# Brochu/RayTrace-WE-GPU

Measured on AMD Instinct MI355X. Metric: Msamples/sec (pixels x spp) at 1920x1080 spp=100 depth=50, higher is better.
Workload: dtype f32

## Files before the change

### raytrace-we-gpu_amd/csrc/rtx_diag.h

```cpp
#pragma once

#include "rtx_internal.h"

#ifndef RTX_DIAG_PROF
#define RTX_DIAG_PROF 0
#endif
#ifndef RTX_DIAG_PIXEL
#define RTX_DIAG_PIXEL 0
#endif
#ifndef RTX_DIAG_COOP
#define RTX_DIAG_COOP 0
#endif
#ifndef RTX_DIAG_RAYS
#define RTX_DIAG_RAYS 0
#endif

namespace rtx {
namespace {

#if RTX_DIAG_PROF
__device__ __forceinline__ uint32_t *diag_slots() {
    __shared__ uint32_t s[4][8];
    return s[(threadIdx.x / 64) & 3u];
}
__device__ __forceinline__ void diag_add(int k, uint32_t v) {
    const uint64_t m = __ballot(1);
    if ((int)(threadIdx.x & 63u) == __ffsll((long long)m) - 1) diag_slots()[k] += v;
}
#define RTX_DIAG_ADD(k, v) diag_add(k, v)
#else
#define RTX_DIAG_ADD(k, v)
#endif

#define RTX_CP(k)                                                   \
    if (RTX_DIAG_COOP && cp) {                                      \
        const unsigned long long tn = __builtin_readcyclecounter(); \
        cp[k] += tn - *tq;                                          \
        *tq = tn;                                                   \
    }

struct Diag {
#if RTX_DIAG_RAYS
    uint32_t rit = 0;
#endif
#if RTX_DIAG_PROF
    unsigned long long pr[7] = {0, 0, 0, 0, 0, 0, 0};
    unsigned long long tq = 0;
#endif
#if RTX_DIAG_COOP
    unsigned long long cpa[8] = {0, 0, 0, 0, 0, 0, 0, 0};
    unsigned long long ctq = 0;
    bool was_coop = false;
#endif
    __device__ __forceinline__ void begin() {
#if RTX_DIAG_PROF
        if ((threadIdx.x & 63u) == 0u)
            for (int k = 0; k < 8; ++k) diag_slots()[k] = 0u;
        tq = __builtin_readcyclecounter();
#endif
#if RTX_DIAG_COOP
        ctq = __builtin_readcyclecounter();
#endif
    }
    __device__ __forceinline__ void section(int k) {
#if RTX_DIAG_PROF
        const unsigned long long tn = __builtin_readcyclecounter();
        pr[k] += tn - tq;
        tq = tn;
#else
        (void)k;
#endif
    }
    __device__ __forceinline__ void iteration(uint64_t act) {
#if RTX_DIAG_PROF
        pr[4]++;
        pr[6] += __popcll(act);
#else
        (void)act;
#endif
    }
    __device__ __forceinline__ void tail_iteration() {
#if RTX_DIAG_PROF
        pr[5]++;
#endif
    }
    __device__ __forceinline__ unsigned long long *coop_begin(uint32_t tier, unsigned long long *&tqp) {
#if RTX_DIAG_COOP
        tqp = &ctq;
        if (tier != (uint32_t)RTX_DIAG_COOP) return nullptr;
        const unsigned long long tn = __builtin_readcyclecounter();
        if (was_coop) cpa[4] += tn - ctq;
        ctq = tn;
        return cpa;
#else
        (void)tier;
        tqp = nullptr;
        return nullptr;
#endif
    }
    __device__ __forceinline__ void coop_end(unsigned long long *cp, uint32_t tier) {
#if RTX_DIAG_COOP
        if (cp) {
            const unsigned long long tn = __builtin_readcyclecounter();
            cpa[3] += tn - ctq;
            ctq = tn;
        }
        was_coop = tier == (uint32_t)RTX_DIAG_COOP;
#else
        (void)cp;
        (void)tier;
#endif
    }
    __device__ __forceinline__ void rays(const KParams &P, f3 o, f3 d, bool live, uint32_t slot) {
#if RTX_DIAG_RAYS
        if (!P.wave_times) return;
        const uint32_t w = blockIdx.x * (blockDim.x / 64u) + threadIdx.x / 64u;
        if ((++rit + w * 13u) % (uint32_t)RTX_DIAG_RAYS != 0u) return;
        unsigned long long r = 0;
        if ((threadIdx.x & 63u) == 0u) r = atomicAdd(&P.wave_times[0], 1ull);
        r = __shfl(r, 0, 64);
        const unsigned long long base = 64ull + 256ull * r;
        if (base + 256ull > 2ull * P.wave_cap) return;
        auto pk = [](float a, float b) {
            return ((unsigned long long)__float_as_uint(b) << 32) | __float_as_uint(a);
        };
        unsigned long long *q = P.wave_times + base + 4u * (threadIdx.x & 63u);
        q[0] = pk(o.x, o.y);
        q[1] = pk(o.z, d.x);
        q[2] = pk(d.y, d.z);
        q[3] = ((unsigned long long)slot << 32) | (live ? 1u : 0u);
#else
        (void)P, (void)o, (void)d, (void)live, (void)slot;
#endif
    }
    __device__ __forceinline__ void finish(const KParams &P) {
#if RTX_DIAG_PROF
        if (P.wave_times && (threadIdx.x & 63u) == 0u) {
            for (int k = 0; k < 7; ++k) atomicAdd(&P.wave_times[k], pr[k]);
            for (int k = 0; k < 7; ++k) atomicAdd(&P.wave_times[8 + k], (unsigned long long)diag_slots()[k]);
        }
#endif
#if RTX_DIAG_COOP
        if (P.wave_times && (threadIdx.x & 63u) == 0u)
            for (int k = 0; k < 6; ++k) atomicAdd(&P.wave_times[k], cpa[k]);
#endif
        (void)P;
    }
};

__device__ __forceinline__ void diag_pixel_start(const KParams &P, uint32_t gid, unsigned long long mode) {
#if RTX_DIAG_PIXEL
    if (P.wave_times && gid < P.wave_cap) P.wave_times[2 * gid] = (__builtin_amdgcn_s_memrealtime() << 2) | mode;
#else
    (void)P;
    (void)gid;
    (void)mode;
#endif
}
__device__ __forceinline__ void diag_pixel_end(const KParams &P, uint32_t gid) {
#if RTX_DIAG_PIXEL
    if (P.wave_times && gid < P.wave_cap) P.wave_times[2 * gid + 1] = __builtin_amdgcn_s_memrealtime();
#else
    (void)P;
    (void)gid;
#endif
}
constexpr bool kDiagAny = RTX_DIAG_PROF || RTX_DIAG_PIXEL || RTX_DIAG_COOP || RTX_DIAG_RAYS;

}
}
```

### raytrace-we-gpu_amd/csrc/rtx_grid.h

```cpp
#pragma once

#include <math.h>
#include <stdint.h>

#include <algorithm>
#include <cmath>
#include <utility>
#include <vector>

#if defined(__HIPCC__)
#define RTX_GD __host__ __device__ __forceinline__
#else
#define RTX_GD static inline
#endif

namespace rtx {

constexpr float kGridOMax = 64.0f;
constexpr double kGridFatCells = 1.0 / 256.0;
constexpr double kGridSlabPad = 1e-3;
#ifndef RTX_GRID_STEPS
#define RTX_GRID_STEPS 48
#endif
#ifndef RTX_GRID_HLOG
#define RTX_GRID_HLOG 0
#endif
constexpr uint32_t kGridMaxSteps = RTX_GRID_STEPS;
constexpr uint32_t kGridMaxCells = 4096;

struct LayerGrid {
    float x0, z0;
    float h, inv_h;
    float ylo, yhi;
    uint32_t nx, nz;
    float far_m;
    uint32_t nblk;
};

template <typename Visit>
RTX_GD bool grid_walk(const LayerGrid &G, uint32_t max_steps, float ox, float oy, float oz, float dx, float dy,
                      float dz, float t_stop, Visit visit) {
    const float o2 = fmaf(ox, ox, fmaf(oy, oy, oz * oz));
    const float d2 = fmaf(dx, dx, fmaf(dy, dy, dz * dz));
    if (!(o2 <= kGridOMax * kGridOMax) || !(d2 <= 3.0e38f)) return false;
    const float inf = INFINITY;
    float t0 = 0.0f, t1 = t_stop >= 0.0f ? t_stop : inf;
    auto clip = [&](float o, float d, float lo, float hi) {
        if (d == 0.0f) {
            if (!(o >= lo && o <= hi)) t1 = -inf;
            return;
        }
        const float inv = 1.0f / d;
        const float ta = (lo - o) * inv, tb = (hi - o) * inv;
        t0 = fmaxf(t0, fminf(ta, tb));
        t1 = fminf(t1, fmaxf(ta, tb));
    };
    clip(oy, dy, G.ylo, G.yhi);
    clip(ox, dx, G.x0, G.x0 + (float)G.nx * G.h);
    clip(oz, dz, G.z0, G.z0 + (float)G.nz * G.h);
    if (!(t0 <= t1)) return true;
    const float sx = (fmaf(t0, dx, ox) - G.x0) * G.inv_h, sz = (fmaf(t0, dz, oz) - G.z0) * G.inv_h;
    int ix = (int)fminf(fmaxf(floorf(sx), 0.0f), (float)(G.nx - 1));
    int iz = (int)fminf(fmaxf(floorf(sz), 0.0f), (float)(G.nz - 1));
    const int stx = dx > 0.0f ? 1 : -1, stz = dz > 0.0f ? 1 : -1;
    const float ivx = dx == 0.0f ? 0.0f : 1.0f / dx, ivz = dz == 0.0f ? 0.0f : 1.0f / dz;
    for (uint32_t k = 0; k < max_steps; ++k) {
        if (!visit((uint32_t)ix * G.nz + (uint32_t)iz)) return false;
        const float bx = fmaf((float)(ix + (dx > 0.0f ? 1 : 0)), G.h, G.x0);
        const float bz = fmaf((float)(iz + (dz > 0.0f ? 1 : 0)), G.h, G.z0);
        const float tx = dx == 0.0f ? inf : (bx - ox) * ivx;
        const float tz = dz == 0.0f ? inf : (bz - oz) * ivz;
        if (!(fminf(tx, tz) <= t1)) return true;
        if (tx <= tz) {
            ix += stx;
            if (ix < 0 || ix >= (int)G.nx) return true;
        } else {
            iz += stz;
            if (iz < 0 || iz >= (int)G.nz) return true;
        }
    }
    return false;
}

template <typename Cell>
RTX_GD uint64_t grid_mask(const LayerGrid &G, Cell cell, float ox, float oy, float oz, float dx, float dy, float dz,
                          float t_stop = INFINITY) {
    uint64_t m = 0ull;
    const bool done = grid_walk(G, kGridMaxSteps, ox, oy, oz, dx, dy, dz, t_stop, [&](uint32_t k) {
        m |= cell(k);
        return true;
    });
    return done ? m : ~0ull;
}

template <typename Add>
inline bool build_layer_grid_cells(const float *sph, uint32_t m, uint32_t max_cells, LayerGrid &G, Add add) {
    if (m == 0) return false;
    const double u = 5.9604644775390625e-08;
    const double y0 = sph[1];
    const double B = 26.0 * u * (double)kGridOMax * (double)kGridOMax;
    auto rho_of = [&](uint32_t j) {
        const double cx = sph[4 * (size_t)j], cz = sph[4 * (size_t)j + 2], r = sph[4 * (size_t)j + 3];
        const double c2 = cx * cx + y0 * y0 + cz * cz;
        return std::sqrt(r * r * (1.0 + 8.0 * u) + 27.0 * u * c2 + B) * (1.0 + 4.0 * u) * (1.0 + 1e-12);
    };
    double rho_max = 0.0, cmax = 0.0, xlo = INFINITY, xhi = -INFINITY, zlo = INFINITY, zhi = -INFINITY;
    for (uint32_t j = 0; j < m; ++j) {
        const double cx = sph[4 * (size_t)j], cz = sph[4 * (size_t)j + 2];
        const double rho = rho_of(j);
        rho_max = std::fmax(rho_max, rho);
        cmax = std::fmax(cmax, std::sqrt(cx * cx + y0 * y0 + cz * cz));
        xlo = std::fmin(xlo, cx - rho), xhi = std::fmax(xhi, cx + rho);
        zlo = std::fmin(zlo, cz - rho), zhi = std::fmax(zhi, cz + rho);
    }
    const double area = std::fmax((xhi - xlo) * (zhi - zlo), 1e-30);
    double h = std::exp2(std::round(std::log2(std::sqrt(area / m))) + RTX_GRID_HLOG);
    while (h < rho_max) h *= 2.0;
    const double fat = kGridFatCells * h;
    const double x0 = (std::floor((xlo - fat) / h) - 1.0) * h, z0 = (std::floor((zlo - fat) / h) - 1.0) * h;
    const double nxd = std::ceil((xhi + fat - x0) / h) + 1.0, nzd = std::ceil((zhi + fat - z0) / h) + 1.0;
    if (nxd * nzd > max_cells || !(std::fabs(x0) < 1e6 && std::fabs(z0) < 1e6)) return false;
    G.nx = (uint32_t)nxd, G.nz = (uint32_t)nzd;
    G.h = (float)h, G.inv_h = (float)(1.0 / h);
    G.x0 = (float)x0, G.z0 = (float)z0;
    const double slab = rho_max + kGridSlabPad;
    G.ylo = nextafterf((float)(y0 - slab), -INFINITY);
    G.yhi = nextafterf((float)(y0 + slab), INFINITY);
    G.far_m = nextafterf((float)(4e-3 * ((double)kGridOMax + cmax) + 1e-3), INFINITY);
    for (uint32_t j = 0; j < m; ++j) {
        const double cx = sph[4 * (size_t)j], cz = sph[4 * (size_t)j + 2];
        const double rho = rho_of(j) + fat;
        const int ax = (int)std::floor((cx - rho - x0) / h), bxi = (int)std::floor((cx + rho - x0) / h);
        const int az = (int)std::floor((cz - rho - z0) / h), bzi = (int)std::floor((cz + rho - z0) / h);
        for (int ix = std::max(ax, 0); ix <= std::min(bxi, (int)G.nx - 1); ++ix)
            for (int iz = std::max(az, 0); iz <= std::min(bzi, (int)G.nz - 1); ++iz) {
                const double qx = std::fmin(std::fmax(cx, x0 + ix * h), x0 + (ix + 1) * h);
                const double qz = std::fmin(std::fmax(cz, z0 + iz * h), z0 + (iz + 1) * h);
                if ((qx - cx) * (qx - cx) + (qz - cz) * (qz - cz) <= rho * rho) add((uint32_t)ix * G.nz + iz, j);
            }
    }
    return true;
}

template <typename Vec>
inline bool build_layer_grid(const float *sph, uint32_t i_lo, uint32_t i_hi, LayerGrid &G, Vec &cell) {
    const uint32_t m = i_hi - i_lo;
    if (m == 0 || (m + 7) / 8 > 64) return false;
    std::vector<std::pair<uint32_t, uint32_t>> hits;
    if (!build_layer_grid_cells(sph + 4 * (size_t)i_lo, m, kGridMaxCells, G,
                                [&](uint32_t k, uint32_t j) { hits.emplace_back(k, j); }))
        return false;
    G.nblk = (m + 7) / 8;
    cell.assign((size_t)G.nx * G.nz, 0ull);
    for (const auto &h : hits) cell[h.first] |= 1ull << (h.second / 8);
    return true;
}

}
```

### raytrace-we-gpu_amd/csrc/rtx_kernels.hip

```cpp
#include <algorithm>
#include <cstdlib>
#include <cstring>
#include <mutex>
#include <type_traits>
#include <vector>

#include "rtx_device_math.h"
#include "rtx_diag.h"
#include "rtx_internal.h"
#include "rtx_prefilter.h"

#if defined(__HIP_DEVICE_COMPILE__) && !defined(__gfx950__)
#error "rtx_kernels.hip targets gfx950 (MI355X) only"
#endif

namespace rtx {

namespace {

constexpr float kTMin = 0.001f;

struct FrameVals {
    f3 org, hor, ver, llc;
    float img_w, img_h;
// ... 383 lines not shown
__device__ __forceinline__ uint32_t scan_prefilter(cfloat_p pre, uint32_t b, uint32_t nblk, const LineTest &T,
                                                   const KScene &S, uint32_t *list, uint32_t &cnt,
                                                   uint32_t *pack = nullptr, const float *lds_pr = nullptr,
                                                   uint64_t gm = ~0ull) {
    cnt = 0;
    uint32_t *my = list + threadIdx.x;
    const LineFlat K = line_test_flat(T, S.flat_cy);
    while (b < nblk) {
        bool full;
        if (b < S.flat_lo) {
            b = scan_range<kPF, false, kTile>(pre, b, min(S.flat_lo, nblk), T, T.nou, T.nov, my, cnt, full, pack, lds_pr);
        } else if (b < S.flat_hi) {
            b = scan_range<kPF, true, kTile>(pre, b, min(S.flat_hi, nblk), T, K.ku, K.kv, my, cnt, full, pack, lds_pr,
                                             gm, S.flat_lo);
        } else {
            b = scan_range<kPF, false, kTile>(pre, b, nblk, T, T.nou, T.nov, my, cnt, full, pack, lds_pr);
        }
        if (full) break;
    }
    return b;
}

__device__ __forceinline__ uint64_t hit_key(float best, int idx) {
    return ((uint64_t)__float_as_uint(best) << 32) | (uint32_t) ~(uint32_t)(idx + 1);
}
__device__ __forceinline__ void key_hit(uint64_t k, float &best, int &idx) {
    best = __uint_as_float((uint32_t)(k >> 32));
    idx = (int)~(uint32_t)k - 1;
}

__device__ __forceinline__ void resolve_one(float4 sc, int g, bool live, f3 o, f3 d, float a, float inv_a,
                                            float t_min, uint64_t &key, bool &ok) {
    const float inf = __uint_as_float(0x7f800000u);
    const float ocx = o.x - sc.x;
    const float ocy = o.y - sc.y;
    const float ocz = o.z - sc.z;
    const float hb = fmaf(ocz, d.z, fmaf(ocy, d.y, ocx * d.x));
    const float cc = fmaf(ocz, ocz, fmaf(ocy, ocy, fmaf(ocx, ocx, -(sc.w * sc.w))));
    const float disc = fmaf(hb, hb, -(a * cc));
    const bool cand = live & !(disc < 0.0f);
    const float sq = sqrt_rn(disc);
    const float rn = (-hb - sq) * inv_a;
    const float rf = (-hb + sq) * inv_a;
    const bool fin = fabsf(rn) < inf && fabsf(rf) < inf;
    ok = ok & (!cand | fin);
    const float c = !(rn < t_min) ? rn : rf;
    const uint64_t k = ((uint64_t)__float_as_uint(c) << 32) | (uint32_t) ~(uint32_t)(g + 1);
    const bool acc = cand & !(c < t_min) & (k < key);
    key = acc ? k : key;
}

struct GiIdentity {
    __device__ __forceinline__ uint32_t operator()(uint32_t p) const { return p; }
};
template <typename Ld, typename Gi = GiIdentity, bool kPos = false>
__device__ __forceinline__ bool resolve_pre_t(Ld ld, uint32_t n, const uint32_t *list, uint32_t m, f3 o, f3 d,
                                              float a, float inv_a, float t_min, float &best, int &idx,
                                              uint32_t cap = (uint32_t)kCand, Gi gi = Gi()) {
    bool ok = true;
    uint32_t j = 0;
    uint32_t e = list[threadIdx.x];
    RTX_DIAG_ADD(4, (uint32_t)__popcll(__ballot(m != 0u)));
#if RTX_DIAG_PROF
    {
        uint32_t c = 0;
        for (uint32_t q = 0; q < m; ++q) c += (uint32_t)__popc(list[min(q, cap) * kRB + threadIdx.x] >> 24);
#pragma unroll
        for (int off = 32; off > 0; off >>= 1) c += (uint32_t)__shfl_xor((int)c, off, 64);
        RTX_DIAG_ADD(5, c);
    }
#endif
    uint32_t pos = 0;
    auto next = [&](uint32_t &i, bool &live) {
        live = j < m;
        pos = (e & 0xffffffu) + (uint32_t)__builtin_ctz(live ? (e >> 24) : 1u);
        if constexpr (kPos) pos = min(pos, n - 1u);
        i = gi(pos);
        e &= e - (1u << 24);
        const bool adv = live && (e >> 24) == 0u;
        j += adv ? 1u : 0u;
        const uint32_t nx = list[min(j, cap) * kRB + threadIdx.x];
        e = adv ? nx : e;
    };
    uint32_t i0;
    bool l0;
    next(i0, l0);
    float4 v0 = kPos ? ld(pos) : ld(min(i0, n - 1u));
    uint64_t key = hit_key(best, idx);
    while (__ballot(l0) != 0ull) {
        RTX_DIAG_ADD(2, 1u);
        uint32_t i1;
        bool l1;
        next(i1, l1);
        const float4 v1 = kPos ? ld(pos) : ld(min(i1, n - 1u));
        resolve_one(v0, (int)i0, l0, o, d, a, inv_a, t_min, key, ok);
        i0 = i1;
        l0 = l1;
        v0 = v1;
    }
    key_hit(key, best, idx);
    return ok;
}
__device__ __forceinline__ bool resolve_pre(const float4 *__restrict__ cen, uint32_t n, const uint32_t *list,
                                            uint32_t m, f3 o, f3 d, float a, float inv_a, float t_min,
                                            float &best, int &idx) {
    return resolve_pre_t([cen](uint32_t i) { return cen[i]; }, n, list, m, o, d, a, inv_a, t_min, best, idx);
}

__device__ __forceinline__ uint32_t scan_culled(const KScene &S, uint32_t b, const LineTest &T, const LineTest &Ts,
                                                const HalfTest &H, const HalfTest &Hs, uint32_t *list,
                                                uint32_t &cnt) {
    cnt = 0;
    uint32_t *my = list + threadIdx.x;
    const uint32_t nblk = S.n_cpad / 8u;
    const LineFlat K = line_test_flat(T, S.flat_cy);
    const LineFlat Ks = line_test_flat(Ts, kCullSy * S.flat_cy);
    const f2v uxs = {Ts.ux, Ts.ux}, uzs = {Ts.uz, Ts.uz}, vzs = {Ts.vz, Ts.vz}, kus = {Ks.ku, Ks.ku},
              kvs = {Ks.kv, Ks.kv};
    const float thr_bs = Ts.thr * kCullThrScaleSy;
    f2v ux = {T.ux, T.ux}, uy = {T.uy, T.uy}, uz = {T.uz, T.uz}, vy = {T.vy, T.vy}, vz = {T.vz, T.vz};
    f2v ku = {K.ku, K.ku}, kv = {K.kv, K.kv};
    const f2v nou = {T.nou, T.nou}, nov = {T.nov, T.nov};
    const f2v th = {T.thr, T.thr};
    const float thr_b = T.thr * kCullThrScale;
    const f2v hdx = {H.dx, H.dx}, hdy = {H.dy, H.dy}, hdz = {H.dz, H.dz}, hnod = {H.nod, H.nod};
    const f2v ha = {H.a, H.a}, htha = {H.tha, H.tha};
    const float kws1 = half_test_kw(Hs, kCullSy * S.flat_cy), kwf1 = half_test_kw(H, S.flat_cy);
    const f2v kwf = {kwf1, kwf1};
    const f2v kws = {kws1, kws1}, has = {Hs.a, Hs.a}, hthas = {Hs.tha, Hs.tha};
    auto quad = [&](auto flat, auto blk, f2v *q) {
#pragma unroll
        for (int p = 0; p < 4; ++p) {
            const f2v cx = {blk(2 * p), blk(2 * p + 1)};
            const f2v cz = {blk(16 + 2 * p), blk(17 + 2 * p)};
            const f2v R = {blk(24 + 2 * p), blk(25 + 2 * p)};
            f2v pu, pv;
            if constexpr (decltype(flat)::value) {
                pu = fma2(cx, ux, fma2(cz, uz, ku));
                pv = fma2(cz, vz, kv);
            } else {
                const f2v cy = {blk(8 + 2 * p), blk(9 + 2 * p)};
                pu = fma2(cx, ux, fma2(cy, uy, fma2(cz, uz, nou)));
                pv = fma2(cy, vy, fma2(cz, vz, nov));
            }
            q[p] = fma2(-pv, pv, fma2(-pu, pu, R));
        }
    };
    auto step = [&](auto flat, uint32_t bb) -> bool {
        const cfloat_p blk = (cfloat_p)S.cpre + 32u * bb;
        float v[32];
#pragma unroll
        for (int i = 0; i < 32; ++i)
            if (!decltype(flat)::value || i < 8 || i >= 16) v[i] = blk[i];
        f2v q[4];
        quad(flat, [&](int i) { return v[i]; }, q);
        const float mx = fmaxf(fmaxf(fmaxf(fmaxf(fmaxf(fmaxf(fmaxf(q[0].x, q[0].y), q[1].x), q[1].y), q[2].x),
                                             q[2].y), q[3].x), q[3].y);
        RTX_DIAG_ADD(0, 1u);
        if (__ballot(!(mx < T.thr)) != 0ull) {
            RTX_DIAG_ADD(1, 1u);
            uint32_t inv = 0;
#pragma unroll
            for (int p = 3; p >= 0; --p) {
                const f2v sq = q[p] - th;
                inv = (inv << 1) | (__float_as_uint(sq.y) >> 31);
                inv = (inv << 1) | (__float_as_uint(sq.x) >> 31);
            }
            uint32_t hm = 0xffu;
            if (RTX_CULL_HALF_SPHERES) {
                hm = 0u;
#pragma unroll
                for (int p = 3; p >= 0; --p) {
                    const f2v cx = {v[2 * p], v[2 * p + 1]}, cz = {v[16 + 2 * p], v[17 + 2 * p]};
                    const f2v R = {v[24 + 2 * p], v[25 + 2 * p]};
                    f2v pw;
                    if constexpr (decltype(flat)::value) {
                        pw = fma2(cx, hdx, fma2(cz, hdz, kwf));
                    } else {
                        const f2v cy = {v[8 + 2 * p], v[9 + 2 * p]};
                        pw = fma2(cx, hdx, fma2(cy, hdy, fma2(cz, hdz, hnod)));
                    }
                    const f2v q2 = fma2(-pw, pw, fma2(R, ha, htha));
                    hm = (hm << 1) | (half_test_pass(pw.y, q2.y) ? 1u : 0u);
                    hm = (hm << 1) | (half_test_pass(pw.x, q2.x) ? 1u : 0u);
                }
            }
            const uint32_t mask = ~inv & hm & 0xffu;
            my[cnt * kRB] = (8u * bb) | (mask << 24);
            cnt += mask != 0u ? 1u : 0u;
            return __ballot(cnt == cand_of<true>()) != 0ull;
        }
        return false;
    };
    using Flat = std::integral_constant<bool, true>;
    using Full = std::integral_constant<bool, false>;
    auto bound_mask1 = [&](cfloat_p grp, bool flat) -> uint32_t {
        float v[32];
        f2v q[4], pw[4], q2[4];
        float thr = thr_b;
        if (flat) {
#pragma unroll
            for (int i = 0; i < 32; ++i)
                if (i < 8 || i >= 16) v[i] = grp[i];
#pragma unroll
            for (int p = 0; p < 4; ++p) {
                const f2v cx = {v[2 * p], v[2 * p + 1]}, cz = {v[16 + 2 * p], v[17 + 2 * p]};
                const f2v R = {v[24 + 2 * p], v[25 + 2 * p]};
                const f2v pu = fma2(cx, uxs, fma2(cz, uzs, kus));
                const f2v pv = fma2(cz, vzs, kvs);
                q[p] = fma2(-pv, pv, fma2(-pu, pu, R));
                pw[p] = fma2(cx, hdx, fma2(cz, hdz, kws));
                q2[p] = fma2(-pw[p], pw[p], fma2(R, has, hthas));
            }
            thr = thr_bs;
        } else {
#pragma unroll
            for (int i = 0; i < 32; ++i) v[i] = grp[i];
            quad(Full(), [&](int i) { return v[i]; }, q);
#pragma unroll
            for (int p = 0; p < 4; ++p) {
                const f2v cx = {v[2 * p], v[2 * p + 1]}, cy = {v[8 + 2 * p], v[9 + 2 * p]};
                const f2v cz = {v[16 + 2 * p], v[17 + 2 * p]}, R = {v[24 + 2 * p], v[25 + 2 * p]};
                pw[p] = fma2(cx, hdx, fma2(cy, hdy, fma2(cz, hdz, hnod)));
                q2[p] = fma2(-pw[p], pw[p], fma2(R, ha, htha));
            }
        }
        uint32_t m = 0;
#pragma unroll
        for (int p = 0; p < 4; ++p) {
            const bool px = !(q[p].x < thr) && (!RTX_CULL_HALF || half_test_pass(pw[p].x, q2[p].x));
            const bool py = !(q[p].y < thr) && (!RTX_CULL_HALF || half_test_pass(pw[p].y, q2[p].y));
            m |= (__ballot(px) != 0ull ? 1u : 0u) << (2 * p);
            m |= (__ballot(py) != 0ull ? 1u : 0u) << (2 * p + 1);
        }
        return m;
    };
    auto first_bits = [](uint32_t n) { return n >= 8u ? 0xffu : (1u << n) - 1u; };
    auto bound_mask = [&](cfloat_p grp, uint32_t b0) -> uint32_t { return bound_mask1(grp, b0 >= S.cflat_lo); };
    const uint32_t ng = (nblk + 7u) / 8u, nsg = (ng + 7u) / 8u, nhg = (nsg + 7u) / 8u;
    for (uint32_t hg = b >> 9; hg < nhg; ++hg) {
        uint32_t m3 = first_bits(nsg - 8u * hg);
        if (RTX_CULL_LEVELS >= 3) m3 &= bound_mask((cfloat_p)S.cbnd3 + 32u * hg, 512u * hg);
        if (hg == (b >> 9)) m3 &= 0xffu << ((b >> 6) & 7u);
        while (m3 != 0u) {
            const uint32_t sg = 8u * hg + (uint32_t)__builtin_ctz(m3);
            m3 &= m3 - 1u;
            uint32_t m2 = bound_mask((cfloat_p)S.cbnd2 + 32u * sg, 64u * sg) & first_bits(ng - 8u * sg);
            if (sg == (b >> 6)) m2 &= 0xffu << ((b >> 3) & 7u);
            RTX_DIAG_ADD(6, (uint32_t)__popc(m2));
            while (m2 != 0u) {
                const uint32_t g = 8u * sg + (uint32_t)__builtin_ctz(m2);
                m2 &= m2 - 1u;
                uint32_t m = bound_mask((cfloat_p)S.cbnd + 32u * g, 8u * g) & first_bits(nblk - 8u * g);
                if (g == (b >> 3)) m &= 0xffu << (b & 7u);
                while (m != 0u) {
                    const uint32_t bb = 8u * g + (uint32_t)__builtin_ctz(m);
                    m &= m - 1u;
                    if (bb >= S.cflat_lo ? step(Flat(), bb) : step(Full(), bb)) return bb + 1u;
                }
            }
        }
    }
    return nblk;
}

__device__ __forceinline__ LineTest line_test_stretched(const KScene &S, f3 o, f3 d) {
    const float dys = kCullSy * d.y;
    const float as = fmaf(d.z, d.z, fmaf(dys, dys, d.x * d.x));
    return line_test_setup(o.x, kCullSy * o.y, o.z, d.x, dys, d.z, as, S.smag * kCullSy);
}
__device__ __forceinline__ HalfTest half_test_stretched(f3 o, f3 d, float thr_bs, float t_min) {
    const float dys = kCullSy * d.y;
    const float as = fmaf(d.z, d.z, fmaf(dys, dys, d.x * d.x));
    return half_test_setup(o.x, kCullSy * o.y, o.z, d.x, dys, d.z, as, thr_bs, t_min);
}
__device__ __forceinline__ int hit_world_culled(const KScene &S, f3 o, f3 d, float a, float inv_a, float t_min,
                                                float &best, uint32_t *list) {
    const LineTest T = line_test_setup(o.x, o.y, o.z, d.x, d.y, d.z, a, S.smag);
    const LineTest Ts = line_test_stretched(S, o, d);
    const HalfTest H = half_test_setup(o.x, o.y, o.z, d.x, d.y, d.z, a, T.thr * kCullThrScale, t_min);
    const HalfTest Hs = half_test_stretched(o, d, Ts.thr * kCullThrScaleSy, t_min);
    const float best0 = best;
    int idx = -1;
    bool ok = true;
    const uint32_t nblk = S.n_cpad / 8u;
    auto ld = [&S](uint32_t p) { return S.ccen[p]; };
    auto gi = [&S](uint32_t p) { return S.cperm[p]; };
    uint32_t b = 0;
    do {
        uint32_t cnt;
        b = scan_culled(S, b, T, Ts, H, Hs, list, cnt);
        ok = resolve_pre_t<decltype(ld), decltype(gi), true>(ld, S.n_cpad, list, cnt, o, d, a, inv_a, t_min, best,
                                                              idx, cand_of<true>(), gi) &&
             ok;
    } while (b < nblk);
    if (!ok) {
        RTX_DIAG_ADD(3, (uint32_t)__popcll(__ballot(1)));
        best = best0;
        idx = hit_blocks_seq((cfloat_p)S.soa, S.n_pad / 8, 0, o, d, a, inv_a, t_min, best, -1);
    }
    return idx;
}

__device__ __forceinline__ uint64_t grid_wave_mask(const KScene &S, f3 o, f3 d, const LineTest &T, uint32_t *spare) {
    const LayerGrid G = *S.grid;
    const uint64_t *gc = reinterpret_cast<const uint64_t *>(S.grid + 1);
    const uint64_t mine = T.thr == -__uint_as_float(0x7f800000u)
                              ? ~0ull
                              : grid_mask(G, [gc](uint32_t k) { return gc[k]; }, o.x, o.y, o.z, d.x, d.y, d.z);
    unsigned long long *w = reinterpret_cast<unsigned long long *>(spare + (threadIdx.x & ~63u));
    const uint32_t lead = (uint32_t)__builtin_amdgcn_readfirstlane((int)threadIdx.x);
    if (threadIdx.x == lead) __hip_atomic_store(w, 0ull, __ATOMIC_RELAXED, __HIP_MEMORY_SCOPE_WORKGROUP);
    __atomic_signal_fence(__ATOMIC_SEQ_CST);
    __hip_atomic_fetch_or(w, (unsigned long long)mine, __ATOMIC_RELAXED, __HIP_MEMORY_SCOPE_WORKGROUP);
    __atomic_signal_fence(__ATOMIC_SEQ_CST);
    const unsigned long long v = __hip_atomic_load(w, __ATOMIC_RELAXED, __HIP_MEMORY_SCOPE_WORKGROUP);
    const uint32_t lo = (uint32_t)__builtin_amdgcn_readfirstlane((int)(uint32_t)v);
    const uint32_t hi = (uint32_t)__builtin_amdgcn_readfirstlane((int)(uint32_t)(v >> 32));
    return ((uint64_t)hi << 32) | lo;
}

template <bool kPF, typename Ld, bool kTile = false, bool kGridOk = true>
__device__ __forceinline__ int hit_world_pre_ld(const KScene &S, Ld ld, f3 o, f3 d, float a, float inv_a,
                                                float t_min, float &best, uint32_t *list, uint32_t *pack = nullptr,
                                                uint32_t start = 0, const float *lds_pr = nullptr,
                                                bool live = true) {
    const cfloat_p pre = (cfloat_p)S.pre;
    const uint32_t nblk = S.n_pad / 8;
    LineTest T = line_test_setup(o.x, o.y, o.z, d.x, d.y, d.z, a, S.smag);
    if (!live) {
        T.ux = T.uy = T.uz = T.vy = T.vz = T.nou = T.nov = 0.0f;
        T.thr = __uint_as_float(0x7f800000u);
    }
    uint64_t gm = ~0ull;
    if constexpr (!kPF && kGridOk) {
        if (RTX_GRID && S.grid != nullptr) gm = grid_wave_mask(S, o, d, T, list + cand_of<kPF>() * kRB);
    }
    const float best0 = best;
    int idx = -1;
    bool ok = true;
    uint32_t b0 = nblk ? start % nblk : 0u;
    if (RTX_PACK && kPF && pack) {
        const uint32_t at = __builtin_amdgcn_readfirstlane(*pack);
        b0 = at < nblk ? (at + nblk - kPackLag) % nblk : 0u;
    }
    uint32_t b = b0, end = nblk;
    for (;;) {
        uint32_t cnt;
        b = scan_prefilter<kPF, kTile>(pre, b, end, T, S, list, cnt, pack, lds_pr, gm);
        ok = resolve_pre_t(ld, S.n, list, cnt, o, d, a, inv_a, t_min, best, idx, cand_of<kPF>()) && ok;
        if (b < end) continue;
        if (end == nblk && b0 != 0u) {
            b = 0;
            end = b0;
            continue;
        }
        break;
    }
    if (!ok) {
        RTX_DIAG_ADD(3, (uint32_t)__popcll(__ballot(1)));
        best = best0;
        idx = hit_blocks_seq((cfloat_p)S.soa, nblk, 0, o, d, a, inv_a, t_min, best, -1);
    }
    return idx;
}
template <bool kPF, bool kGridOk = true>
__device__ __forceinline__ int hit_world_pre(const KScene &S, f3 o, f3 d, float a, float inv_a,
                                             float t_min, float &best, uint32_t *list, uint32_t *pack = nullptr,
                                             uint32_t start = 0) {
    const float4 *__restrict__ cen = S.cen;
    auto ld = [cen](uint32_t i) { return cen[i]; };
    return hit_world_pre_ld<kPF, decltype(ld), false, kGridOk>(S, ld, o, d, a, inv_a, t_min, best, list, pack, start);
}

constexpr uint32_t kCoopSlots = 32;
constexpr uint32_t kCoopWaveBytes = kCoopSlots * 10 * sizeof(float);
constexpr uint32_t kCoopBytes = (kRB / 64) * kCoopWaveBytes;
constexpr uint32_t kCoopLds = 640;
constexpr uint32_t kCoopPad = 128;
static_assert(kCoopMax <= (int)kCoopSlots, "kCoopMax must be <= 32");
__host__ __device__ constexpr uint32_t coop_npad(uint32_t n) { return (n + kCoopPad - 1u) / kCoopPad * kCoopPad; }
__host__ __device__ constexpr uint32_t coop_lds_bytes(uint32_t n) {
    return coop_npad(n) * 4u * (uint32_t)sizeof(float) + n * (uint32_t)sizeof(float);
}
static_assert(coop_lds_bytes(kCoopLds) <= 12800, "LDS copy of the scene: 5 render blocks per CU");

struct SphLds {
    static constexpr bool kPadded = true;
    const float *pr;
    const float *rad;
    uint32_t n, npairs;
    __device__ __forceinline__ void pair(uint32_t p, f2v &cx, f2v &cy, f2v &cz, f2v &R) const {
        const float4 *q = reinterpret_cast<const float4 *>(pr + 8u * p);
        const float4 a = q[0], b = q[1];
        cx = f2v{a.x, a.y};
        cy = f2v{a.z, a.w};
        cz = f2v{b.x, b.y};
        R = f2v{b.z, b.w};
    }
    __device__ __forceinline__ float4 sphere(uint32_t j) const {
        const float *q = pr + 8u * (j >> 1) + (j & 1u);
        return make_float4(q[0], q[2], q[4], rad[min(j, n - 1u)]);
    }
};
struct SphGlobal {
    static constexpr bool kPadded = false;
    const float *pre;
    const float4 *cen;
    uint32_t n, npairs;
    __device__ __forceinline__ void pair(uint32_t p, f2v &cx, f2v &cy, f2v &cz, f2v &R) const {
        const float *b = pre + 32u * (p >> 2) + 2u * (p & 3u);
        cx = *reinterpret_cast<const f2v *>(b);
        cy = *reinterpret_cast<const f2v *>(b + 8);
        cz = *reinterpret_cast<const f2v *>(b + 16);
        R = *reinterpret_cast<const f2v *>(b + 24);
    }
    __device__ __forceinline__ float4 sphere(uint32_t j) const { return cen[min(j, n - 1u)]; }
};

__device__ __forceinline__ SphLds lds_copy(const KScene &S, float *base, bool on, uint32_t nthreads = kRB) {
    SphLds l;
    l.n = S.n;
    l.npairs = coop_npad(S.n) / 2u;
    l.pr = base;
    l.rad = base + 8u * l.npairs;
    if (on) {
        float *pr = base, *rad = base + 8u * l.npairs;
        for (uint32_t i = threadIdx.x; i < 2u * l.npairs; i += nthreads) {
            const float4 c = S.pre4[min(i, S.n - 1u)];
            float *q = pr + 8u * (i >> 1) + (i & 1u);
            q[0] = c.x;
            q[2] = c.y;
            q[4] = c.z;
            q[6] = c.w;
            if (i < S.n) rad[i] = S.cen[i].w;
        }
    }
    return l;
}
__device__ __forceinline__ SphGlobal sph_global(const KScene &S) {
    SphGlobal g;
    g.pre = S.pre;
    g.cen = S.cen;
    g.n = S.n;
    g.npairs = S.n_pad / 2u;
    return g;
}

template <bool kMax>
__device__ __forceinline__ uint32_t group_reduce_u32(uint32_t v, uint32_t lg) {
    auto op = [](uint32_t x, uint32_t y) { return kMax ? max(x, y) : min(x, y); };
    if (lg >= 1u) v = op(v, (uint32_t)__builtin_amdgcn_update_dpp(0, (int)v, 0xB1, 0xF, 0xF, false));
    if (lg >= 2u) v = op(v, (uint32_t)__builtin_amdgcn_update_dpp(0, (int)v, 0x4E, 0xF, 0xF, false));
    if (lg >= 3u) v = op(v, (uint32_t)__builtin_amdgcn_update_dpp(0, (int)v, 0x141, 0xF, 0xF, false));
    if (lg >= 4u) v = op(v, (uint32_t)__builtin_amdgcn_update_dpp(0, (int)v, 0x140, 0xF, 0xF, false));
    if (lg >= 5u) {
        const auto r = __builtin_amdgcn_permlane16_swap(v, v, false, false);
        v = op((uint32_t)r[0], (uint32_t)r[1]);
    }
    if (lg >= 6u) {
        const auto r = __builtin_amdgcn_permlane32_swap(v, v, false, false);
        v = op((uint32_t)r[0], (uint32_t)r[1]);
    }
    return v;
}

constexpr uint32_t kGfRays = 32;
static_assert(kGfRays * 10 * sizeof(float) <= kCoopWaveBytes, "coop scratch: 8 floats per ray + 2 result words");
#ifndef RTX_GF_STEPS
#define RTX_GF_STEPS 16
#endif
constexpr uint32_t kGfSteps = RTX_GF_STEPS;
static_assert(kGfSteps >= 1 && kGfSteps <= 16, "flag mask: 2 bits per step in 32");
template <typename Src>
__device__ __forceinline__ int hit_world_groups(const KScene &S, const Src &src, uint64_t act, bool active, f3 o, f3 d,
                                                float a, float inv_a, float t_min, float *ws, float &best, bool &seq,
                                                unsigned long long *cp = nullptr, unsigned long long *tq = nullptr) {
    const uint32_t lane = threadIdx.x & 63u;
    const uint32_t m_all = (uint32_t)__popcll(act);
    const uint32_t rank_all =
        __builtin_amdgcn_mbcnt_hi((uint32_t)(act >> 32), __builtin_amdgcn_mbcnt_lo((uint32_t)act, 0u));
    uint32_t *keys = reinterpret_cast<uint32_t *>(ws + 8 * kGfRays);
    const float inf = __uint_as_float(0x7f800000u);
    int result = -1;
    seq = false;
#pragma unroll 1
    for (uint32_t c0 = 0; c0 < m_all; c0 += kGfRays) {
        const uint32_t m = min(m_all - c0, kGfRays);
        const bool mine = active && rank_all >= c0 && rank_all < c0 + m;
        const uint32_t rank = rank_all - c0;
        if (mine) {
            float *w = ws + 8 * rank;
            w[0] = o.x;
            w[1] = o.y;
            w[2] = o.z;
            w[3] = d.x;
            w[4] = d.y;
            w[5] = d.z;
            w[6] = a;
            w[7] = inv_a;
        }
        __builtin_amdgcn_wave_barrier();
        if (RTX_DIAG_COOP && cp && c0 == 0u) cp[5]++;
        RTX_CP(0)
        const uint32_t lg = m <= 1u ? 6u : 6u - (32u - (uint32_t)__builtin_clz(m - 1u));
        const uint32_t g = 1u << lg;
        const uint32_t r = lane >> lg, k = lane & (g - 1u);
        const bool valid = r < m;
        const float *w = ws + 8 * (valid ? r : 0u);
        const f3 ro = mk3(w[0], w[1], w[2]), rd = mk3(w[3], w[4], w[5]);
        const float ra = w[6], ria = w[7];
        const LineTest T = line_test_setup(ro.x, ro.y, ro.z, rd.x, rd.y, rd.z, ra, S.smag);
        const f2v ux = {T.ux, T.ux}, uy = {T.uy, T.uy}, uz = {T.uz, T.uz}, vy = {T.vy, T.vy}, vz = {T.vz, T.vz};
        const f2v nou = {T.nou, T.nou}, nov = {T.nov, T.nov}, th = {T.thr, T.thr};
        uint64_t key = hit_key(inf, -1);
        bool ok = true;
        const uint32_t nsteps = valid ? (src.npairs + g - 1u) >> lg : 0u;
        const uint32_t plast = src.npairs - 1u;
#pragma unroll 1
        for (uint32_t s0 = 0; __ballot(s0 < nsteps) != 0ull; s0 += kGfSteps) {
            uint32_t im = 0;
            const uint32_t s1 = min(s0 + kGfSteps, nsteps);
            auto step = [&](uint32_t st) {
                f2v cx, cy, cz, R;
                src.pair(Src::kPadded ? (st << lg) + k : min((st << lg) + k, plast), cx, cy, cz, R);
                const f2v pu = fma2(cx, ux, fma2(cy, uy, fma2(cz, uz, nou)));
                const f2v pv = fma2(cy, vy, fma2(cz, vz, nov));
                const f2v q = fma2(-pv, pv, fma2(-pu, pu, R)) - th;
                im = (im << 1) | (__float_as_uint(q.y) >> 31);
                im = (im << 1) | (__float_as_uint(q.x) >> 31);
            };
            uint32_t st = s0;
            for (; st + 2u <= s1; st += 2u) {
                step(st);
                step(st + 1u);
            }
            if (st < s1) step(st);
            const uint32_t nb = 2u * (s1 > s0 ? s1 - s0 : 0u);
            uint32_t fm = ~im & (nb >= 32u ? ~0u : ((1u << nb) - 1u));
#pragma unroll 1
            while (__ballot(fm != 0u) != 0ull) {
                const bool live = fm != 0u;
                const uint32_t bit = live ? (uint32_t)__builtin_ctz(fm) : 0u;
                fm &= fm - 1u;
                const uint32_t p = ((s1 - 1u - (bit >> 1)) << lg) + k;
                const uint32_t j = 2u * (Src::kPadded ? p : min(p, plast)) + (bit & 1u);
                resolve_one(src.sphere(j), (int)j, live, ro, rd, ra, ria, t_min, key, ok);
            }
        }
        RTX_CP(1)
        const uint32_t cb0 = (uint32_t)(key >> 32);
        const uint32_t cb = group_reduce_u32<false>(cb0, lg);
        const uint32_t ib = group_reduce_u32<true>(cb0 == cb ? ~(uint32_t)key : 0u, lg);
        const uint64_t badm = __ballot(!ok);
        if (valid && k == 0u) {
            const uint64_t gm = (g == 64u ? ~0ull : ((1ull << g) - 1ull)) << (r * g);
            keys[2 * r] = (badm & gm) != 0ull ? 0xffffffffu : ib;
            keys[2 * r + 1] = cb;
        }
        __builtin_amdgcn_wave_barrier();
        RTX_CP(2)
        if (mine) {
            const uint32_t kb = keys[2 * rank], kc = keys[2 * rank + 1];
            if (kb == 0xffffffffu) {
                seq = true;
            } else if (kb != 0u) {
                const float c = __uint_as_float(kc);
                if (c <= best) {
                    best = c;
                    result = (int)(kb - 1u);
                }
            }
        }
        __builtin_amdgcn_wave_barrier();
    }
    return active ? result : -1;
}

template <bool kBfs = true>
__device__ __forceinline__ int hit_world_groups_culled(const KScene &S, uint64_t act, bool active, f3 o, f3 d,
                                                       float a, float inv_a, float t_min, float *ws, float &best,
                                                       bool &seq) {
    const uint32_t lane = threadIdx.x & 63u;
    const uint32_t m_all = (uint32_t)__popcll(act);
    const uint32_t rank_all =
        __builtin_amdgcn_mbcnt_hi((uint32_t)(act >> 32), __builtin_amdgcn_mbcnt_lo((uint32_t)act, 0u));
    uint32_t *keys = reinterpret_cast<uint32_t *>(ws + 8 * kGfRays);
    const float inf = __uint_as_float(0x7f800000u);
    const uint32_t nblk = S.n_cpad / 8u, ngrp = (nblk + 7u) / 8u;
    int result = -1;
    seq = false;
#pragma unroll 1
    for (uint32_t c0 = 0; c0 < m_all; c0 += kGfRays) {
        const uint32_t m = min(m_all - c0, kGfRays);
        const bool mine = active && rank_all >= c0 && rank_all < c0 + m;
        const uint32_t rank = rank_all - c0;
        if (mine) {
            float *w = ws + 8 * rank;
            w[0] = o.x;
            w[1] = o.y;
            w[2] = o.z;
            w[3] = d.x;
            w[4] = d.y;
            w[5] = d.z;
            w[6] = a;
            w[7] = inv_a;
        }
        __builtin_amdgcn_wave_barrier();
        const uint32_t lg = m <= 1u ? 6u : 6u - (32u - (uint32_t)__builtin_clz(m - 1u));
        const uint32_t g = 1u << lg;
        const uint32_t r = lane >> lg, k = lane & (g - 1u);
        const bool valid = r < m;
        const float *w = ws + 8 * (valid ? r : 0u);
        const f3 ro = mk3(w[0], w[1], w[2]), rd = mk3(w[3], w[4], w[5]);
        const float ra = w[6], ria = w[7];
        const LineTest T = line_test_setup(ro.x, ro.y, ro.z, rd.x, rd.y, rd.z, ra, S.smag);
        const LineTest Ts = line_test_stretched(S, ro, rd);
        const float thr_b = T.thr * kCullThrScale, thr_bs = Ts.thr * kCullThrScaleSy;
        const HalfTest H = half_test_setup(ro.x, ro.y, ro.z, rd.x, rd.y, rd.z, ra, thr_b, t_min);
        const HalfTest Hs = half_test_stretched(ro, rd, thr_bs, t_min);
        auto block_mask = [&](const float *blk, const LineTest &L, float thr,
                              const HalfTest *Hh = nullptr) -> uint32_t {
            const f2v ux = {L.ux, L.ux}, uy = {L.uy, L.uy}, uz = {L.uz, L.uz}, vy = {L.vy, L.vy}, vz = {L.vz, L.vz};
            const f2v nou = {L.nou, L.nou}, nov = {L.nov, L.nov};
            const float4 *b4 = reinterpret_cast<const float4 *>(blk);
            float4 v[8];
#pragma unroll
            for (int t = 0; t < 8; ++t) v[t] = b4[t];
            uint32_t msk = 0;
#pragma unroll
            for (int p = 0; p < 4; ++p) {
                const float4 X = v[p >> 1], Y = v[2 + (p >> 1)], Z = v[4 + (p >> 1)], Rr = v[6 + (p >> 1)];
                const bool hi = p & 1;
                const f2v cx = {hi ? X.z : X.x, hi ? X.w : X.y}, cy = {hi ? Y.z : Y.x, hi ? Y.w : Y.y};
                const f2v cz = {hi ? Z.z : Z.x, hi ? Z.w : Z.y}, R = {hi ? Rr.z : Rr.x, hi ? Rr.w : Rr.y};
                const f2v pu = fma2(cx, ux, fma2(cy, uy, fma2(cz, uz, nou)));
                const f2v pv = fma2(cy, vy, fma2(cz, vz, nov));
                const f2v q = fma2(-pv, pv, fma2(-pu, pu, R));
                bool px = !(q.x < thr), py = !(q.y < thr);
                if (RTX_CULL_HALF && Hh) {
                    const f2v hdx = {Hh->dx, Hh->dx}, hdy = {Hh->dy, Hh->dy}, hdz = {Hh->dz, Hh->dz};
                    const f2v hnod = {Hh->nod, Hh->nod}, ha = {Hh->a, Hh->a}, htha = {Hh->tha, Hh->tha};
                    const f2v pw = fma2(cx, hdx, fma2(cy, hdy, fma2(cz, hdz, hnod)));
                    const f2v q2 = fma2(-pw, pw, fma2(R, ha, htha));
                    px = px && half_test_pass(pw.x, q2.x);
                    py = py && half_test_pass(pw.y, q2.y);
                }
                msk |= (px ? 1u : 0u) << (2 * p);
                msk |= (py ? 1u : 0u) << (2 * p + 1);
            }
            return msk;
        };
        auto bound_pass = [&](const float *q, bool flat) -> bool {
// ... 1962 lines not shown
```

Baseline: 6229.

## Distribute grid cell-mask walk across wave lanes instead of per-lane DDA

Each lane now computes the slab of grid columns its ray crosses (a 'stretch'). The wave prefix-sums the per-lane column counts and assigns one column per lane per round, so every active lane fetches up to three cell masks for whichever ray owns that work item. Ownership is shared through LDS marks and ds_bpermute. The grid header is also loaded through a scalar (constant-address) pointer. This replaces the divergent per-lane DDA walk with balanced cooperative loads, at the cost of extra ballots, LDS traffic and permutes per round. It adds optional profiling counters as well.

```diff
diff --git a/raytrace-we-gpu_amd/csrc/rtx_diag.h b/raytrace-we-gpu_amd/csrc/rtx_diag.h
--- a/raytrace-we-gpu_amd/csrc/rtx_diag.h
+++ b/raytrace-we-gpu_amd/csrc/rtx_diag.h
@@ -28,8 +28,40 @@
     if ((int)(threadIdx.x & 63u) == __ffsll((long long)m) - 1) diag_slots()[k] += v;
 }
 #define RTX_DIAG_ADD(k, v) diag_add(k, v)
+__device__ __forceinline__ unsigned long long *diag_hw() {
+    __shared__ unsigned long long s[4][8];
+    return s[(threadIdx.x / 64) & 3u];
+}
+__device__ __forceinline__ void diag_hw_clock(int k) {
+    const uint64_t m = __ballot(1);
+    if ((int)(threadIdx.x & 63u) == __ffsll((long long)m) - 1) {
+        const unsigned long long tn = __builtin_readcyclecounter();
+        if (k >= 0) diag_hw()[k] += tn - diag_hw()[3];
+        diag_hw()[3] = tn;
+    }
+}
+__device__ __forceinline__ void diag_hw_walk(uint32_t steps, uint32_t rounds) {
+    uint32_t mx = 0;
+    for (int b = 7; b >= 0; --b) {
+        const uint32_t t = mx | (1u << b);
+        if (__ballot(min(steps, 255u) >= t) != 0ull) mx = t;
+    }
+    const uint64_t m = __ballot(1);
+    if ((int)(threadIdx.x & 63u) == __ffsll((long long)m) - 1) {
+        diag_hw()[4] += 1ull;
+        diag_hw()[5] += mx;
+        diag_hw()[7] += rounds ? rounds : mx;
+    }
+    atomicAdd(&diag_hw()[6], (unsigned long long)steps);
+}
+#define RTX_DIAG_HW_BEGIN() diag_hw_clock(-1)
+#define RTX_DIAG_HW(k) diag_hw_clock(k)
+#define RTX_DIAG_WALK(steps, rounds) diag_hw_walk(steps, rounds)
 #else
 #define RTX_DIAG_ADD(k, v)
+#define RTX_DIAG_HW_BEGIN()
+#define RTX_DIAG_HW(k)
+#define RTX_DIAG_WALK(steps, rounds)
 #endif
 
 #define RTX_CP(k)                                                   \
@@ -55,7 +87,7 @@
     __device__ __forceinline__ void begin() {
 #if RTX_DIAG_PROF
         if ((threadIdx.x & 63u) == 0u)
-            for (int k = 0; k < 8; ++k) diag_slots()[k] = 0u;
+            for (int k = 0; k < 8; ++k) diag_slots()[k] = 0u, diag_hw()[k] = 0ull;
         tq = __builtin_readcyclecounter();
 #endif
 #if RTX_DIAG_COOP
@@ -138,6 +170,8 @@
         if (P.wave_times && (threadIdx.x & 63u) == 0u) {
             for (int k = 0; k < 7; ++k) atomicAdd(&P.wave_times[k], pr[k]);
             for (int k = 0; k < 7; ++k) atomicAdd(&P.wave_times[8 + k], (unsigned long long)diag_slots()[k]);
+            if (P.wave_cap >= 12u)
+                for (int k = 0; k < 8; ++k) atomicAdd(&P.wave_times[16 + k], diag_hw()[k]);
         }
 #endif
 #if RTX_DIAG_COOP
diff --git a/raytrace-we-gpu_amd/csrc/rtx_grid.h b/raytrace-we-gpu_amd/csrc/rtx_grid.h
--- a/raytrace-we-gpu_amd/csrc/rtx_grid.h
+++ b/raytrace-we-gpu_amd/csrc/rtx_grid.h
@@ -93,6 +93,103 @@
     return done ? m : ~0ull;
 }
 
+#ifndef RTX_GRID_COOP_EPS
+#define RTX_GRID_COOP_EPS (1.0f / 64.0f)
+#endif
+constexpr float kGridCoopEps = RTX_GRID_COOP_EPS;
+
+RTX_GD float grid_clampf(float x, float lo, float hi) {
+#if defined(__HIP_DEVICE_COMPILE__)
+    return __builtin_amdgcn_fmed3f(x, lo, hi);
+#else
+    return fminf(fmaxf(x, lo), hi);
+#endif
+}
+
+struct GridStretch {
+    float lo, hi, A, s;
+    uint32_t c0, n, zmajor;
+};
+
+RTX_GD bool grid_stretch(const LayerGrid &G, float ox, float oy, float oz, float dx, float dy, float dz,
+                         GridStretch &R) {
+    R.lo = R.hi = R.A = R.s = 0.0f;
+    R.c0 = R.n = R.zmajor = 0u;
+    const float o2 = fmaf(ox, ox, fmaf(oy, oy, oz * oz));
+    const float d2 = fmaf(dx, dx, fmaf(dy, dy, dz * dz));
+    if (!(o2 <= kGridOMax * kGridOMax) || !(d2 <= 3.0e38f)) return false;
+    const float inf = INFINITY;
+    float t0 = 0.0f, t1 = inf;
+    auto clip = [&](float o, float d, float lo, float hi) {
+        if (d == 0.0f) {
+            if (!(o >= lo && o <= hi)) t1 = -inf;
+            return 0.0f;
+        }
+        const float inv = 1.0f / d;
+        const float ta = (lo - o) * inv, tb = (hi - o) * inv;
+        t0 = fmaxf(t0, fminf(ta, tb));
+        t1 = fminf(t1, fmaxf(ta, tb));
+        return inv;
+    };
+    clip(oy, dy, G.ylo, G.yhi);
+    const float ivx = clip(ox, dx, G.x0, G.x0 + (float)G.nx * G.h);
+    const float ivz = clip(oz, dz, G.z0, G.z0 + (float)G.nz * G.h);
+    if (!(t0 <= t1)) return true;
+    if (!(t1 <= 3.0e38f)) return false;
+    const bool zm = fabsf(dz) > fabsf(dx);
+    const float om = zm ? oz : ox, dm = zm ? dz : dx, on = zm ? ox : oz, dn = zm ? dx : dz;
+    const float M0 = zm ? G.z0 : G.x0, N0 = zm ? G.x0 : G.z0;
+    const float nM = (float)(zm ? G.nz : G.nx);
+    const float s = dn * (zm ? ivz : ivx);
+    if (!(fabsf(s) <= 2.0f)) return false;
+    const float a0 = (fmaf(t0, dm, om) - M0) * G.inv_h, a1 = (fmaf(t1, dm, om) - M0) * G.inv_h;
+    const float b0 = (fmaf(t0, dn, on) - N0) * G.inv_h;
+    R.lo = fminf(a0, a1), R.hi = fmaxf(a0, a1);
+    R.s = s;
+    R.A = fmaf(-a0, s, b0);
+    const float c0 = grid_clampf(floorf(R.lo - kGridCoopEps), 0.0f, nM - 1.0f);
+    const float c1 = grid_clampf(floorf(R.hi + kGridCoopEps), 0.0f, nM - 1.0f);
+    R.c0 = (uint32_t)c0;
+    R.zmajor = zm ? 1u : 0u;
+    const uint32_t n = (uint32_t)c1 - (uint32_t)c0 + 1u;
+    if (n > kGridMaxSteps) return false;
+    R.n = n;
+    return true;
+}
+
+RTX_GD void grid_item_cells(const LayerGrid &G, float lo, float hi, float A, float s, uint32_t zmajor, uint32_t c,
+                            uint32_t &k0, uint32_t &stride, uint32_t &cnt) {
+    const float ma = grid_clampf((float)c, lo, hi), mb = grid_clampf((float)(c + 1u), lo, hi);
+    const float na = fmaf(ma, s, A), nb = fmaf(mb, s, A);
+    const float nN = (float)(zmajor ? G.nx : G.nz);
+    const float j0 = grid_clampf(floorf(fminf(na, nb) - kGridCoopEps), 0.0f, nN - 1.0f);
+    const float j1 = grid_clampf(floorf(fmaxf(na, nb) + kGridCoopEps), 0.0f, nN - 1.0f);
+    const uint32_t j = (uint32_t)j0;
+    const uint32_t w = (uint32_t)j1 - j + 1u;
+    cnt = w < 3u ? w : 3u;
+    k0 = zmajor ? j * G.nz + c : c * G.nz + j;
+    stride = zmajor ? G.nz : 1u;
+}
+
+template <typename Cell>
+RTX_GD uint64_t grid_mask_items(const LayerGrid &G, Cell cell, float ox, float oy, float oz, float dx, float dy,
+                                float dz) {
+    GridStretch R;
+    if (!grid_stretch(G, ox, oy, oz, dx, dy, dz, R)) return ~0ull;
+    uint64_t m = 0ull;
+    for (uint32_t i = 0; i < R.n; ++i) {
+        uint32_t k0, stride, cnt;
+        grid_item_cells(G, R.lo, R.hi, R.A, R.s, R.zmajor, R.c0 + i, k0, stride, cnt);
+        for (uint32_t q = 0; q < cnt; ++q) m |= cell(k0 + q * stride);
+    }
+    return m;
+}
+
+RTX_GD int grid_share_mark(uint32_t start, uint32_t n, uint32_t base, uint32_t nact) {
+    if (n == 0u || start + n <= base || start >= base + nact) return -1;
+    return (int)(start > base ? start - base : 0u);
+}
+
 template <typename Add>
 inline bool build_layer_grid_cells(const float *sph, uint32_t m, uint32_t max_cells, LayerGrid &G, Add add) {
     if (m == 0) return false;
diff --git a/raytrace-we-gpu_amd/csrc/rtx_kernels.hip b/raytrace-we-gpu_amd/csrc/rtx_kernels.hip
--- a/raytrace-we-gpu_amd/csrc/rtx_kernels.hip
+++ b/raytrace-we-gpu_amd/csrc/rtx_kernels.hip
@@ -709,15 +709,85 @@
     return idx;
 }
 
-__device__ __forceinline__ uint64_t grid_wave_mask(const KScene &S, f3 o, f3 d, const LineTest &T, uint32_t *spare) {
-    const LayerGrid G = *S.grid;
-    const uint64_t *gc = reinterpret_cast<const uint64_t *>(S.grid + 1);
-    const uint64_t mine = T.thr == -__uint_as_float(0x7f800000u)
-                              ? ~0ull
-                              : grid_mask(G, [gc](uint32_t k) { return gc[k]; }, o.x, o.y, o.z, d.x, d.y, d.z);
+__device__ __forceinline__ uint64_t grid_wave_mask(const KScene &S, f3 o, f3 d, const LineTest &T, uint32_t *list,
+                                                   uint32_t *spare) {
+    typedef const __attribute__((address_space(4))) LayerGrid *grid_cp;
+    typedef const __attribute__((address_space(1))) uint64_t *cell_gp;
+    const uint64_t ga = (uint64_t)(uintptr_t)S.grid;
+    uint32_t alo = (uint32_t)ga, ahi = (uint32_t)(ga >> 32);
+    asm volatile("" : "+v"(alo), "+v"(ahi));
+    alo = (uint32_t)__builtin_amdgcn_readfirstlane((int)alo);
+    ahi = (uint32_t)__builtin_amdgcn_readfirstlane((int)ahi);
+    const uint64_t gaddr = ((uint64_t)ahi << 32) | alo;
+    const grid_cp gp = (grid_cp)(uintptr_t)gaddr;
+    LayerGrid G;
+    G.x0 = gp->x0, G.z0 = gp->z0, G.h = gp->h, G.inv_h = gp->inv_h, G.ylo = gp->ylo, G.yhi = gp->yhi;
+    G.nx = gp->nx, G.nz = gp->nz, G.far_m = 0.0f, G.nblk = 0u;
+    const cell_gp gc = (cell_gp)(uintptr_t)(gaddr + sizeof(LayerGrid));
+    GridStretch R;
+    const bool mine_ok =
+        T.thr != -__uint_as_float(0x7f800000u) && grid_stretch(G, o.x, o.y, o.z, d.x, d.y, d.z, R);
+    if (__ballot(!mine_ok) != 0ull) {
+        RTX_DIAG_WALK(0u, 1u);
+        return ~0ull;
+    }
+    const uint32_t lane = threadIdx.x & 63u;
+    const uint64_t act = __ballot(1);
+    auto below = [](uint64_t m) {
+        return __builtin_amdgcn_mbcnt_hi((uint32_t)(m >> 32), __builtin_amdgcn_mbcnt_lo((uint32_t)m, 0u));
+    };
+    const uint32_t nact = (uint32_t)__popcll(act), slot = below(act);
+    static_assert(kGridMaxSteps < 64u, "grid_wave_mask: item counts of 6 bits");
+    uint32_t start = 0, total = 0;
+#pragma unroll
+    for (uint32_t b = 0; b < 6u; ++b) {
+        const uint64_t mb = __ballot(((R.n >> b) & 1u) != 0u);
+        start += below(mb) << b;
+        total += (uint32_t)__popcll(mb) << b;
+    }
+    const uint32_t pack = start | (R.c0 << 12) | (R.zmajor << 24);
+    static_assert(63u * kGridMaxSteps < 4096u && kGridMaxCells <= 4096u, "grid_wave_mask: packed owner word");
+    const uint32_t last_cell = G.nx * G.nz - 1u;
+    uint32_t *marks = list + (threadIdx.x & ~63u);
+    uint32_t *my_mark = marks + slot;
+    auto from = [](uint32_t lane4, uint32_t v) {
+        return (uint32_t)__builtin_amdgcn_ds_bpermute((int)lane4, (int)v);
+    };
+    uint64_t mine = 0ull;
+    uint32_t rounds = 0;
+    for (uint32_t base = 0; base < total; base += nact) {
+        ++rounds;
+        __hip_atomic_store(my_mark, 0u, __ATOMIC_RELAXED, __HIP_MEMORY_SCOPE_WORKGROUP);
+        __atomic_signal_fence(__ATOMIC_SEQ_CST);
+        const int ms = grid_share_mark(start, R.n, base, nact);
+        if (ms >= 0)
+            __hip_atomic_store(marks + ms, lane + 1u, __ATOMIC_RELAXED, __HIP_MEMORY_SCOPE_WORKGROUP);
+        __atomic_signal_fence(__ATOMIC_SEQ_CST);
+        const uint32_t v = __hip_atomic_load(my_mark, __ATOMIC_RELAXED, __HIP_MEMORY_SCOPE_WORKGROUP);
+        __atomic_signal_fence(__ATOMIC_SEQ_CST);
+        const uint64_t le = __ballot(v != 0u) & ((2ull << lane) - 1ull);
+        const bool valid = base + slot < total;
+        const uint32_t at = le != 0ull ? 63u - (uint32_t)__clzll((long long)le) : lane;
+        const uint32_t own4 = ((from(4u * at, v) - 1u) & 63u) * 4u;
+        const uint32_t opack = from(own4, pack);
+        const float olo = __uint_as_float(from(own4, __float_as_uint(R.lo)));
+        const float ohi = __uint_as_float(from(own4, __float_as_uint(R.hi)));
+        const float oA = __uint_as_float(from(own4, __float_as_uint(R.A)));
+        const float os = __uint_as_float(from(own4, __float_as_uint(R.s)));
+        if (valid) {
+            const uint32_t c = ((opack >> 12) & 0xfffu) + (base + slot - (opack & 0xfffu));
+            uint32_t k0, stride, cnt;
+            grid_item_cells(G, olo, ohi, oA, os, opack >> 24, c, k0, stride, cnt);
+            const uint64_t m0 = gc[min(k0, last_cell)];
+            const uint64_t m1 = gc[min(k0 + (cnt > 1u ? stride : 0u), last_cell)];
+            mine |= m0 | m1;
+            if (cnt > 2u) mine |= gc[min(k0 + 2u * stride, last_cell)];
+        }
+    }
+    RTX_DIAG_WALK(R.n, rounds);
+    (void)rounds;
     unsigned long long *w = reinterpret_cast<unsigned long long *>(spare + (threadIdx.x & ~63u));
-    const uint32_t lead = (uint32_t)__builtin_amdgcn_readfirstlane((int)threadIdx.x);
-    if (threadIdx.x == lead) __hip_atomic_store(w, 0ull, __ATOMIC_RELAXED, __HIP_MEMORY_SCOPE_WORKGROUP);
+    if (slot == 0u) __hip_atomic_store(w, 0ull, __ATOMIC_RELAXED, __HIP_MEMORY_SCOPE_WORKGROUP);
     __atomic_signal_fence(__ATOMIC_SEQ_CST);
     __hip_atomic_fetch_or(w, (unsigned long long)mine, __ATOMIC_RELAXED, __HIP_MEMORY_SCOPE_WORKGROUP);
     __atomic_signal_fence(__ATOMIC_SEQ_CST);
@@ -734,6 +804,7 @@
                                                 bool live = true) {
     const cfloat_p pre = (cfloat_p)S.pre;
     const uint32_t nblk = S.n_pad / 8;
+    RTX_DIAG_HW_BEGIN();
     LineTest T = line_test_setup(o.x, o.y, o.z, d.x, d.y, d.z, a, S.smag);
     if (!live) {
         T.ux = T.uy = T.uz = T.vy = T.vz = T.nou = T.nov = 0.0f;
@@ -741,8 +812,9 @@
     }
     uint64_t gm = ~0ull;
     if constexpr (!kPF && kGridOk) {
-        if (RTX_GRID && S.grid != nullptr) gm = grid_wave_mask(S, o, d, T, list + cand_of<kPF>() * kRB);
-    }
+        if (RTX_GRID && S.grid != nullptr) gm = grid_wave_mask(S, o, d, T, list, list + cand_of<kPF>() * kRB);
+    }
+    RTX_DIAG_HW(0);
     const float best0 = best;
     int idx = -1;
     bool ok = true;
@@ -755,7 +827,9 @@
     for (;;) {
         uint32_t cnt;
         b = scan_prefilter<kPF, kTile>(pre, b, end, T, S, list, cnt, pack, lds_pr, gm);
+        RTX_DIAG_HW(1);
         ok = resolve_pre_t(ld, S.n, list, cnt, o, d, a, inv_a, t_min, best, idx, cand_of<kPF>()) && ok;
+        RTX_DIAG_HW(2);
         if (b < end) continue;
         if (end == nblk && b0 != 0u) {
             b = 0;
```

Result: faster. 6486, median of 6 (+4.1%).
